# gfacciol/mgm

Hardware: AMD Instinct MI355X
Metric: disparity-volumes/sec (W*H*L cost volume -> 8-dir MGM -> WTA+vfit) (higher is better)
Workload: dtype f32

## Files before the change

### mgm_amd/csrc/mgm_wta.hip

```cpp
#include <algorithm>
#include <cstdlib>

#include "mgm_device.h"
#include "mgm_planner.h"

namespace mgm {

__device__ __forceinline__ void vfit(float v0, float v1, float v2, float &v_min, float &x_min)
{
    if ((v1 > v0) && (v1 > v2)) {
        v_min = v1;
        x_min = 0.0f;
        return;
    }
    float slope = v2 - v1;
    if ((v2 - v1) < (v0 - v1)) slope = v0 - v1;
    x_min = (v0 - v2) / (2.0f * slope);
    v_min = v2 + (x_min - 1.0f) * slope;
}

template <int LPL, int PPW, bool EXACT, int MAXD = kMaxDirs, int SUB = 1>
__global__ void __launch_bounds__(256) k_wta(const WtaParams P)
{
    static_assert(SUB == 1 || EXACT, "several pixels per slab only without padding lanes");
    constexpr int LP = LPL * 64;
    constexpr int LANES = 64 / SUB;
    __shared__ float sS[4][LP];
    const int wv = threadIdx.x >> 6, lane = threadIdx.x & 63;
    const int L = P.L;
    const int Lr_ = P.Lreal;
    constexpr bool exact = EXACT;
    const int Ls = SUB > 1 ? LP : L;
    const int m0 = lane * LPL;
    const int sub = lane / LANES;
    const int o0 = (lane % LANES) * LPL;
    const bool c8 = P.C8 && exact;
    const long long nslab = P.npix / SUB;
    for (long long g0 = ((long long)blockIdx.x * 4 + wv) * PPW; g0 < nslab; g0 += (long long)gridDim.x * 4 * PPW) {
        float c[PPW][LPL], l[MAXD][PPW][LPL];
#pragma unroll
        for (int u = 0; u < PPW; u++) {
            const long long g = g0 + u < nslab ? g0 + u : nslab - 1;
            if (c8 && P.cbytes == 2) {
                const unsigned short *q = reinterpret_cast<const unsigned short *>(P.C8) + g * Ls + m0;
#pragma unroll
                for (int k = 0; k < LPL; k++) c[u][k] = c16_decode(q[k]);
            } else if (c8) {
                const uint8_t *q = P.C8 + g * Ls + m0;
#pragma unroll
                for (int k = 0; k < LPL; k++) c[u][k] = c8_decode(q[k]);
            } else {
                const float *q = P.C + g * Ls + m0;
#pragma unroll
                for (int k = 0; k < LPL; k++) c[u][k] = (exact || m0 + k < L) ? q[k] : f_inf();
            }
        }
#pragma unroll
        for (int p = 0; p < MAXD; p++) {
            if (p < P.NDIR) {
#pragma unroll
                for (int u = 0; u < PPW; u++) {
                    const long long g = g0 + u < nslab ? g0 + u : nslab - 1;
                    const float *q = P.Lr + (long long)p * P.nvol + g * Ls + m0;
#pragma unroll
                    for (int k = 0; k < LPL; k++) l[p][u][k] = (exact || m0 + k < L) ? q[k] : f_inf();
                }
            }
        }
#pragma unroll
        for (int u = 0; u < PPW; u++) {
            if (g0 + u >= nslab) break;
            const long long pix = (g0 + u) * SUB + sub;
            float S[LPL];
#pragma unroll
            for (int k = 0; k < LPL; k++) S[k] = 0.0f;
#pragma unroll
            for (int p = 0; p < MAXD; p++) {
                if (p < P.NDIR) {
#pragma unroll
                    for (int k = 0; k < LPL; k++) S[k] = S[k] + l[p][u][k];
                }
            }
            if (P.FIX == 1) {
                const float f = (float)(P.NDIR - 1);
#pragma unroll
                for (int k = 0; k < LPL; k++) S[k] = S[k] - f * c[u][k];
            }
            float vout = 0.0f;
            if (P.FIX == 1) vout = vout - (float)(P.NDIR - 1) * f_inf();
            if (P.clo) {
                const int cl = (int)P.clo[pix] - P.dmin, ch = (int)P.chi[pix] - P.dmin;
#pragma unroll
                for (int k = 0; k < LPL; k++)
                    if (o0 + k < cl || o0 + k > ch) S[k] = vout;
            }
            if (P.S) {
                float *q = P.S + pix * Lr_ + o0;
#pragma unroll
                for (int k = 0; k < LPL; k++)
                    if (o0 + k < Lr_) q[k] = S[k];
            }
            float best = f_inf();
            int bi = 0x7fffffff;
            const bool windowed = P.wlo != nullptr;
            int wl = 0, wh = 0;
            if (windowed) {
                wl = (int)P.wlo[pix] - P.dmin;
                wh = (int)P.whi[pix] - P.dmin;
            }
#pragma unroll
            for (int k = 0; k < LPL; k++) {
                const float v = S[k];
                if (o0 + k < Lr_ && (!windowed || (o0 + k >= wl && o0 + k <= wh)) && finite_bits(v) && best > v) {
                    best = v;
                    bi = o0 + k;
                }
            }
#pragma unroll
            for (int d = LANES / 2; d >= 1; d >>= 1) {
                const float ov = __shfl_xor(best, d);
                const int oi = __shfl_xor(bi, d);
                if (ov < best || (ov == best && oi < bi)) {
                    best = ov;
                    bi = oi;
                }
            }
            if (windowed) {
                if (finite_bits(vout)) {
                    if (wl < 0 && wl <= wh && !(best < vout)) {
                        best = vout;
                        bi = wl;
                    }
                    const int hi0 = wl > Lr_ ? wl : Lr_;
                    if (wh >= Lr_ && hi0 <= wh && vout < best) {
                        best = vout;
                        bi = hi0;
                    }
                }
            }
            float outv, outc = best;
            if (bi == 0x7fffffff) outv = __builtin_nanf("");
            else outv = (float)(bi + P.dmin);
            if (P.refine == 1 && !windowed) {
#pragma unroll
                for (int k = 0; k < LPL; k++) sS[wv][m0 + k] = S[k];
                asm volatile("s_waitcnt lgkmcnt(0)" ::: "memory");
                if (bi != 0x7fffffff && bi - 1 >= 0 && bi + 2 <= Lr_ - 1) {
                    const float *sp = sS[wv] + sub * L;
                    const float v0 = sp[bi - 1], v1 = sp[bi], v2 = sp[bi + 1];
                    float vmin, dx;
                    vfit(v0, v1, v2, vmin, dx);
                    outv = (float)(bi + P.dmin) + dx;
                    outc = vmin;
                }
                asm volatile("s_waitcnt lgkmcnt(0)" ::: "memory");
            }
            if (lane % LANES == 0) {
                P.out[pix] = outv;
                P.outcost[pix] = outc;
            }
        }
    }
}

template <int L, int MAXD>
__global__ void __launch_bounds__(256) k_wta_q(const WtaParams P)
{
    static_assert(L == 192 || L == 384, "groups of 768 floats");
    constexpr int NPX = 768 / L;
    constexpr int CPP = L / 4;
    __shared__ float sS[4][768];
    const int wv = threadIdx.x >> 6, lane = threadIdx.x & 63;
    const bool c8 = P.C8 != nullptr;
    const long long ngroup = P.npix / NPX;
    int cpix[3], clab[3];
#pragma unroll
    for (int j = 0; j < 3; j++) {
        const int t = 64 * j + lane;
        cpix[j] = t / CPP;
        clab[j] = (t % CPP) * 4;
    }
    for (long long g = (long long)blockIdx.x * 4 + wv; g < ngroup; g += (long long)gridDim.x * 4) {
        float c[3][4], l[MAXD][3][4];
#pragma unroll
        for (int j = 0; j < 3; j++) {
            if (c8 && P.cbytes == 2) {
                const uint2 w = *reinterpret_cast<const uint2 *>(P.C8 + (g * 768 + 256 * j + 4 * lane) * 2);
                c[j][0] = c16_decode(w.x & 65535u); c[j][1] = c16_decode(w.x >> 16);
                c[j][2] = c16_decode(w.y & 65535u); c[j][3] = c16_decode(w.y >> 16);
            } else if (c8) {
                const unsigned w = *reinterpret_cast<const unsigned *>(P.C8 + g * 768 + 256 * j + 4 * lane);
#pragma unroll
                for (int k = 0; k < 4; k++) c[j][k] = c8_decode((w >> (8 * k)) & 255u);
            } else {
                const float4 q = *reinterpret_cast<const float4 *>(P.C + g * 768 + 256 * j + 4 * lane);
                c[j][0] = q.x; c[j][1] = q.y; c[j][2] = q.z; c[j][3] = q.w;
            }
        }
#pragma unroll
        for (int p = 0; p < MAXD; p++)
            if (p < P.NDIR) {
#pragma unroll
                for (int j = 0; j < 3; j++) {
                    const float4 q = *reinterpret_cast<const float4 *>(P.Lr + (long long)p * P.nvol + g * 768 + 256 * j + 4 * lane);
                    l[p][j][0] = q.x; l[p][j][1] = q.y; l[p][j][2] = q.z; l[p][j][3] = q.w;
                }
            }
        float S[3][4];
        const float f = (float)(P.NDIR - 1);
#pragma unroll
        for (int j = 0; j < 3; j++)
#pragma unroll
            for (int k = 0; k < 4; k++) {
                float a = 0.0f;
#pragma unroll
                for (int p = 0; p < MAXD; p++)
                    if (p < P.NDIR) a = a + l[p][j][k];
                if (P.FIX == 1) a = a - f * c[j][k];
                S[j][k] = a;
            }
        if (P.S) {
#pragma unroll
            for (int j = 0; j < 3; j++) *reinterpret_cast<float4 *>(P.S + g * 768 + 256 * j + 4 * lane) = make_float4(S[j][0], S[j][1], S[j][2], S[j][3]);
        }
        float cb[3];
        int ci[3];
#pragma unroll
        for (int j = 0; j < 3; j++) {
            cb[j] = f_inf();
            ci[j] = 0x7fffffff;
#pragma unroll
            for (int k = 0; k < 4; k++)
                if (finite_bits(S[j][k]) && cb[j] > S[j][k]) {
                    cb[j] = S[j][k];
                    ci[j] = clab[j] + k;
                }
        }
        if (P.refine == 1) {
#pragma unroll
            for (int j = 0; j < 3; j++) *reinterpret_cast<float4 *>(&sS[wv][256 * j + 4 * lane]) = make_float4(S[j][0], S[j][1], S[j][2], S[j][3]);
        }
#pragma unroll
        for (int q = 0; q < NPX; q++) {
            float best = f_inf();
            int bi = 0x7fffffff;
#pragma unroll
            for (int j = 0; j < 3; j++)
                if (cpix[j] == q && (cb[j] < best)) {
                    best = cb[j];
                    bi = ci[j];
                }
#pragma unroll
            for (int d = 32; d >= 1; d >>= 1) {
                const float ov = __shfl_xor(best, d);
                const int oi = __shfl_xor(bi, d);
                if (ov < best || (ov == best && oi < bi)) {
                    best = ov;
                    bi = oi;
                }
            }
            float outv, outc = best;
            if (bi == 0x7fffffff) outv = __builtin_nanf("");
            else outv = (float)(bi + P.dmin);
            if (P.refine == 1) {
                asm volatile("s_waitcnt lgkmcnt(0)" ::: "memory");
                if (bi != 0x7fffffff && bi - 1 >= 0 && bi + 2 <= L - 1) {
                    const float *sp = sS[wv] + q * L;
                    float vmin, dx;
                    vfit(sp[bi - 1], sp[bi], sp[bi + 1], vmin, dx);
                    outv = (float)(bi + P.dmin) + dx;
                    outc = vmin;
                }
            }
            if (lane == 0) {
                P.out[g * NPX + q] = outv;
                P.outcost[g * NPX + q] = outc;
            }
        }
        if (P.refine == 1) asm volatile("s_waitcnt lgkmcnt(0)" ::: "memory");
    }
}

__global__ void __launch_bounds__(256) k_wta_any(const WtaParams P)
{
    const int wv = threadIdx.x >> 6, lane = threadIdx.x & 63;
    const int L = P.L, Lr_ = P.Lreal;
    const float f = (float)(P.NDIR - 1);
    float vout = 0.0f;
    if (P.FIX == 1) vout = vout - f * f_inf();
    for (long long pix = (long long)blockIdx.x * 4 + wv; pix < P.npix; pix += (long long)gridDim.x * 4) {
        int cl = 0, ch = Lr_ - 1;
        if (P.clo) {
            cl = (int)P.clo[pix] - P.dmin;
            ch = (int)P.chi[pix] - P.dmin;
        }
        const bool windowed = P.wlo != nullptr;
        int wl = 0, wh = 0;
        if (windowed) {
            wl = (int)P.wlo[pix] - P.dmin;
            wh = (int)P.whi[pix] - P.dmin;
        }
        auto S_at = [&](int o) {
            float a = 0.0f;
            for (int p = 0; p < P.NDIR; p++) a = a + P.Lr[(long long)p * P.nvol + pix * L + o];
            if (P.FIX == 1)
                a = a - f * (!P.C8 ? P.C[pix * L + o]
                                   : (P.cbytes == 2 ? c16_decode(reinterpret_cast<const unsigned short *>(P.C8)[pix * L + o]) : c8_decode(P.C8[pix * L + o])));
            if (o < cl || o > ch) a = vout;
            return a;
        };
        float best = f_inf();
        int bi = 0x7fffffff;
        for (int o = lane; o < Lr_; o += 64) {
            const float v = S_at(o);
            if (P.S) P.S[pix * Lr_ + o] = v;
            if ((!windowed || (o >= wl && o <= wh)) && finite_bits(v) && best > v) {
                best = v;
                bi = o;
            }
        }
#pragma unroll
        for (int d = 32; d >= 1; d >>= 1) {
            const float ov = __shfl_xor(best, d);
            const int oi = __shfl_xor(bi, d);
            if (ov < best || (ov == best && oi < bi)) {
                best = ov;
                bi = oi;
            }
        }
        if (windowed && finite_bits(vout)) {
            if (wl < 0 && wl <= wh && !(best < vout)) {
                best = vout;
                bi = wl;
            }
            const int hi0 = wl > Lr_ ? wl : Lr_;
            if (wh >= Lr_ && hi0 <= wh && vout < best) {
                best = vout;
                bi = hi0;
            }
        }
        float outv, outc = best;
        if (bi == 0x7fffffff) outv = __builtin_nanf("");
        else outv = (float)(bi + P.dmin);
        if (P.refine == 1 && !windowed && bi != 0x7fffffff && bi - 1 >= 0 && bi + 2 <= Lr_ - 1) {
            float vmin, dx;
            vfit(S_at(bi - 1), S_at(bi), S_at(bi + 1), vmin, dx);
            outv = (float)(bi + P.dmin) + dx;
            outc = vmin;
        }
        if (lane == 0) {
            P.out[pix] = outv;
            P.outcost[pix] = outc;
        }
    }
}

template <int MAXD>
__device__ __forceinline__ void sum_fix(const float (&l)[MAXD][4], const float (&c)[4], int ndir, int fix, float (&S)[4])
{
#pragma unroll
    for (int k = 0; k < 4; k++) S[k] = 0.0f;
#pragma unroll
    for (int p = 0; p < MAXD; p++)
        if (p < ndir) {
#pragma unroll
            for (int k = 0; k < 4; k++) S[k] = S[k] + l[p][k];
        }
    if (fix == 1) {
        const float f = (float)(ndir - 1);
#pragma unroll
        for (int k = 0; k < 4; k++) S[k] = S[k] - f * c[k];
    }
}
template <int CTRL>
__device__ __forceinline__ float dpp_fmin(float v)
{
    return __builtin_fminf(v, __builtin_bit_cast(float, __builtin_amdgcn_update_dpp(0, __builtin_bit_cast(int, v), CTRL, 0xf, 0xf, false)));
}
template <int PPW, int MAXD, bool ALLD>
__global__ void __launch_bounds__(256) k_wta_pruned(const WtaParams P)
{
    constexpr int L = 256;
    __shared__ float sS[4][PPW][L];
    const int wv = threadIdx.x >> 6, lane = threadIdx.x & 63;
    const int ch = lane >> 3;
    const int o0 = lane * 4;
    const int ndir = ALLD ? MAXD : P.NDIR, fix = P.FIX;
    const long long mstride = P.nvol / 32;
    unsigned nloaded = 0, npx = 0;
    for (long long g0 = ((long long)blockIdx.x * 4 + wv) * PPW; g0 < P.npix; g0 += (long long)gridDim.x * 4 * PPW) {
        unsigned cw[PPW];
        float mn[PPW][MAXD];
#pragma unroll
        for (int u = 0; u < PPW; u++) {
            const long long pix = g0 + u < P.npix ? g0 + u : P.npix - 1;
            cw[u] = *reinterpret_cast<const unsigned *>(P.C8 + pix * L + o0);
#pragma unroll
            for (int p = 0; p < MAXD; p++)
                if (p < ndir) mn[u][p] = P.Lmin[(long long)p * mstride + pix * (L / 32) + ch];
        }
        float c[PPW][4], clb[PPW];
        int seed[PPW];
#pragma unroll
        for (int u = 0; u < PPW; u++) {
            float lm[MAXD][4], LB[4];
#pragma unroll
            for (int k = 0; k < 4; k++) c[u][k] = c8_decode((cw[u] >> (8 * k)) & 255u);
#pragma unroll
            for (int p = 0; p < MAXD; p++)
#pragma unroll
                for (int k = 0; k < 4; k++) lm[p][k] = p < ndir ? mn[u][p] : 0.0f;
            sum_fix<MAXD>(lm, c[u], ndir, fix, LB);
            float lb = f_inf();
#pragma unroll
            for (int k = 0; k < 4; k++) lb = c[u][k] < f_inf() ? __builtin_fminf(lb, LB[k]) : lb;
            lb = lb == lb ? lb : -f_inf();
            lb = dpp_fmin<0xB1>(lb);
            lb = dpp_fmin<0x4E>(lb);
            lb = dpp_fmin<0x141>(lb);
            clb[u] = lb;
            const float gmin = wave_min(lb);
            const unsigned long long at = __builtin_amdgcn_ballot_w64(lb == gmin);
            seed[u] = gmin < f_inf() ? (int)(__builtin_ctzll(at) >> 3) : -1;
        }
        float S[PPW][4];
        bool act[PPW];
        float best0[PPW];
        {
            float l[PPW][MAXD][4];
#pragma unroll
            for (int u = 0; u < PPW; u++) {
                const long long pix = g0 + u < P.npix ? g0 + u : P.npix - 1;
                act[u] = ch == seed[u];
                const float *q0 = P.Lr + pix * L + (seed[u] > 0 ? seed[u] : 0) * 32 + (lane & 7) * 4;
#pragma unroll
                for (int p = 0; p < MAXD; p++)
                    if (p < ndir) {
                        const float4 q = *reinterpret_cast<const float4 *>(q0 + (long long)p * P.nvol);
                        l[u][p][0] = q.x, l[u][p][1] = q.y, l[u][p][2] = q.z, l[u][p][3] = q.w;
                    }
            }
#pragma unroll
            for (int u = 0; u < PPW; u++) {
                sum_fix<MAXD>(l[u], c[u], ndir, fix, S[u]);
                float b = f_inf();
#pragma unroll
                for (int k = 0; k < 4; k++) b = (act[u] && finite_bits(S[u][k]) && S[u][k] < b) ? S[u][k] : b;
                best0[u] = wave_min(b);
            }
        }
        bool act2[PPW];
        {
            float l[PPW][MAXD][4];
#pragma unroll
            for (int u = 0; u < PPW; u++) {
                const long long pix = g0 + u < P.npix ? g0 + u : P.npix - 1;
                act2[u] = !act[u] && seed[u] >= 0 && clb[u] <= best0[u];
                const float *q0 = P.Lr + pix * L + (act2[u] ? ch : (seed[u] > 0 ? seed[u] : 0)) * 32 + (lane & 7) * 4;
#pragma unroll
                for (int p = 0; p < MAXD; p++)
                    if (p < ndir) {
                        const float4 q = *reinterpret_cast<const float4 *>(q0 + (long long)p * P.nvol);
                        l[u][p][0] = q.x, l[u][p][1] = q.y, l[u][p][2] = q.z, l[u][p][3] = q.w;
                    }
            }
#pragma unroll
            for (int u = 0; u < PPW; u++) {
                float S2[4];
                sum_fix<MAXD>(l[u], c[u], ndir, fix, S2);
#pragma unroll
                for (int k = 0; k < 4; k++) S[u][k] = act[u] ? S[u][k] : S2[k];
            }
        }
#pragma unroll
        for (int u = 0; u < PPW; u++) {
            if (g0 + u >= P.npix) break;
            const long long pix = g0 + u;
            const bool have = act[u] || act2[u];
            const unsigned long long lmask = __builtin_amdgcn_ballot_w64(have);
            nloaded += (unsigned)__builtin_popcountll(lmask & 0x0101010101010101ull);
            npx++;
            float best = f_inf();
            int bi = 0x7fffffff;
            if (have) {
#pragma unroll
                for (int k = 0; k < 4; k++)
                    if (finite_bits(S[u][k]) && best > S[u][k]) {
                        best = S[u][k];
                        bi = o0 + k;
                    }
            }
            const float gbest = wave_min(best);
            const unsigned long long who = __builtin_amdgcn_ballot_w64(bi != 0x7fffffff && best == gbest);
            best = gbest;
            bi = who ? __builtin_amdgcn_readlane(bi, (int)__builtin_ctzll(who)) : 0x7fffffff;
            float outv, outc = best;
            if (bi == 0x7fffffff) outv = __builtin_nanf("");
            else outv = (float)(bi + P.dmin);
            if (P.refine == 1) {
                if (have) {
#pragma unroll
                    for (int k = 0; k < 4; k++) sS[wv][u][o0 + k] = S[u][k];
                }
                if (bi != 0x7fffffff && bi - 1 >= 0 && bi + 2 <= L - 1) {
                    auto S_at = [&](int o) -> float {
                        if ((lmask >> ((o >> 5) * 8)) & 1ull) return sS[wv][u][o];
                        float a = 0.0f;
                        for (int p = 0; p < ndir; p++) a = a + P.Lr[(long long)p * P.nvol + pix * L + o];
                        if (fix == 1) a = a - (float)(ndir - 1) * c8_decode(P.C8[pix * L + o]);
                        return a;
                    };
                    const float v0 = S_at(bi - 1), v1 = S_at(bi), v2 = S_at(bi + 1);
                    float vmin, dx;
                    vfit(v0, v1, v2, vmin, dx);
                    outv = (float)(bi + P.dmin) + dx;
                    outc = vmin;
                }
            }
            if (lane == 0) {
                P.out[pix] = outv;
                P.outcost[pix] = outc;
            }
        }
    }
    if (P.stats && lane == 0) atomicAdd(P.stats + (blockIdx.x & 63) * 16, ((unsigned long long)npx << 32) | nloaded);
}

static_assert(kWtaWidestLabels == kMaxLPL * 64, "plan_wta sends wider volumes to k_wta_any");
hipError_t launch_wta(const WtaParams &p, const WtaChoice &c, hipStream_t s)
{
    const dim3 grid((unsigned)c.grid), block(256);
#define WTA(LPL_, PPW_, EXACT_, MAXD_, SUB_)                                                                     \
    if (c.LPL == LPL_ && c.PPW == PPW_ && c.EXACT == EXACT_ && c.MAXD == MAXD_ && c.SUB == SUB_) {               \
        hipLaunchKernelGGL((k_wta<LPL_, PPW_, EXACT_ != 0, MAXD_, SUB_>), grid, block, 0, s, p);                 \
        return hipGetLastError();                                                                                \
    }
#define WTA_Q(LPL_, MAXD_)                                                                                       \
    if (c.LPL == LPL_ && c.MAXD == MAXD_) {                                                                      \
        hipLaunchKernelGGL((k_wta_q<64 * LPL_, MAXD_>), grid, block, 0, s, p);                                   \
        return hipGetLastError();                                                                                \
    }
#define WTA_PRUNED(PPW_, MAXD_, ALLD_)                                                                           \
    if (c.PPW == PPW_ && c.MAXD == MAXD_ && c.ALLD == ALLD_) {                                                   \
        hipLaunchKernelGGL((k_wta_pruned<PPW_, MAXD_, ALLD_ != 0>), grid, block, 0, s, p);                       \
        return hipGetLastError();                                                                                \
    }
    switch (c.family) {
        case kWtaPruned:
            if (!p.Lmin) break;
            WTA_PRUNED(2, 8, 1) WTA_PRUNED(1, 8, 1) WTA_PRUNED(2, 4, 1) WTA_PRUNED(1, 4, 1) WTA_PRUNED(1, 4, 0) WTA_PRUNED(1, 8, 0)
            break;
        case kWtaAny:
            hipLaunchKernelGGL(k_wta_any, grid, block, 0, s, p);
            return hipGetLastError();
        case kWtaQuad:
            WTA_Q(3, 4) WTA_Q(3, 8) WTA_Q(6, 4) WTA_Q(6, 8)
            break;
        case kWtaPacked:
            WTA(4, 4, 1, 4, 2) WTA(4, 2, 1, 8, 2) WTA(4, 4, 1, 4, 4) WTA(4, 2, 1, 8, 4)
            break;
        case kWtaPlain:
            WTA(1, 8, 1, 4, 1) WTA(1, 4, 1, 8, 1) WTA(1, 1, 0, 8, 1)
            WTA(2, 8, 1, 4, 1) WTA(2, 4, 1, 8, 1) WTA(2, 1, 0, 8, 1)
            WTA(3, 4, 1, 4, 1) WTA(3, 2, 1, 8, 1) WTA(3, 1, 0, 8, 1)
            WTA(4, 6, 1, 4, 1) WTA(4, 3, 1, 8, 1) WTA(4, 1, 0, 8, 1)
            WTA(6, 2, 1, 4, 1) WTA(6, 1, 1, 8, 1) WTA(6, 1, 0, 8, 1)
            WTA(8, 2, 1, 4, 1) WTA(8, 1, 1, 8, 1) WTA(8, 1, 0, 8, 1)
            WTA(12, 1, 1, 8, 1) WTA(12, 1, 0, 8, 1)
            WTA(16, 1, 1, 8, 1) WTA(16, 1, 0, 8, 1)
            WTA(24, 1, 0, 8, 1)
            WTA(32, 1, 0, 8, 1)
            break;
        default: break;
    }
#undef WTA
#undef WTA_Q
#undef WTA_PRUNED
    return hipErrorInvalidValue;
}

__device__ __forceinline__ void parabolafit(const float (&v)[4], float &v_min, float &x_min)
{
    if (v[1] > v[0] && v[1] > v[2]) {
        x_min = 0;
        v_min = v[1];
        return;
    }
    const float c = v[1];
    const float b = (v[2] - v[0]) / 2;
    const float a = (v[2] - 2 * v[1] + v[0]) / 2;
    float x = -b / (2 * a);
    if (x > 1) x = 1;
    if (x < -1) x = -1;
    v_min = (a * x + b) * x + c;
    x_min = x;
}

__device__ __forceinline__ void parabolafit_ocv(const float (&v)[4], float &v_min, float &x_min)
{
    if (v[1] > v[0] && v[1] > v[2]) {
        x_min = 0;
        v_min = v[1];
        return;
    }
    const float c = v[1];
    float b = (v[2] - v[0]) / 2;
    float a = (v[2] - 2 * v[1] + v[0]) / 2;
    a *= 2;
    b *= 2;
    a = a > 1.0 ? a : 1.0;
    float x = (-b + a) / (2 * a);
    if (x > 1) x = 1;
    if (x < -1) x = -1;
    v_min = (a * x + b) * x + c;
    x_min = x;
}

__device__ __forceinline__ float cubic_interp(const float (&p)[4], const float x)
{
    return p[1] + 0.5 * x *
                      (p[2] - p[0] + x * (2.0 * p[0] - 5.0 * p[1] + 4.0 * p[2] - p[3] + x * (3.0 * (p[1] - p[2]) + p[3] - p[0])));
}

__device__ __forceinline__ void cubicfit(const float (&p)[4], float &out_pmin, float &out_xmin)
{
    float pmin, xmin;
    if (p[1] < p[2]) {
        pmin = p[1];
        xmin = 0.0;
    } else {
        pmin = p[2];
        xmin = 1.0;
    }
    const double a = 0.5 * 3.0 * (3.0 * (p[1] - p[2]) + p[3] - p[0]);
    const double b = 2.0 * p[0] - 5.0 * p[1] + 4.0 * p[2] - p[3];
    const double c = 0.5 * (p[2] - p[0]);
    const double discr = b * b - 4.0 * a * c;
    if (discr >= 0) {
        const double z1 = (-b + __builtin_sqrt(discr)) / (2.0 * a);
        const double z2 = (-b - __builtin_sqrt(discr)) / (2.0 * a);
        if (z1 > 0.0 && z1 < 1.0) {
            const float tmp = cubic_interp(p, z1);
            if (tmp < pmin) {
                pmin = tmp;
                xmin = z1;
            }
        }
        if (z2 > 0.0 && z2 < 1.0) {
            const float tmp = cubic_interp(p, z2);
            if (tmp < pmin) {
                pmin = tmp;
                xmin = z2;
            }
        }
    }
    out_pmin = pmin;
    out_xmin = xmin;
}

template <int SPL, int CB>
__global__ void __launch_bounds__(256) k_wta_rel(const WtaRelParams P)
{
    constexpr int SLOTS = 16 * SPL;
    const int wv = threadIdx.x >> 6, lane = threadIdx.x & 63, li = lane & 15, grp = lane >> 4;
    const float f = (float)(P.NDIR - 1);
    float vout = 0.0f;
    if (P.FIX == 1) vout = vout - f * f_inf();
    const bool vfin = finite_bits(vout);
    const long long nquads = (P.npix + 3) / 4;
    for (long long q4 = (long long)blockIdx.x * 4 + wv; q4 < nquads; q4 += (long long)gridDim.x * 4) {
        const long long pix0 = q4 * 4 + grp;
        const bool live = pix0 < P.npix;
        const long long pix = live ? pix0 : P.npix - 1;
        const int4 rec = reinterpret_cast<const int4 *>(P.base)[pix];
        const int b = rec.x, lo = rec.y, hi = rec.z;
        const bool windowed = P.wlo != nullptr;
        const int wl = windowed ? (int)P.wlo[pix] : lo, wh = windowed ? (int)P.whi[pix] : hi;
        typedef float f4 __attribute__((ext_vector_type(4)));
        float a[SPL];
#pragma unroll
        for (int q = 0; q < SPL; q++) a[q] = 0.0f;
        for (int p = 0; p < P.NDIR; p++) {
#pragma unroll
            for (int h = 0; h < SPL / 4; h++) {
                const f4 t = reinterpret_cast<const f4 *>(P.Lr + (long long)p * P.nvol + pix * SLOTS + SPL * li)[h];
#pragma unroll
                for (int q = 0; q < 4; q++) a[4 * h + q] = a[4 * h + q] + t[q];
            }
        }
        if (P.FIX == 1) {
            constexpr int NWORD = SPL * CB / 4;
            unsigned cw[NWORD];
#pragma unroll
            for (int w = 0; w < NWORD; w++) cw[w] = reinterpret_cast<const unsigned *>(P.c8 + (pix * SLOTS + SPL * li) * CB)[w];
#pragma unroll
            for (int q = 0; q < SPL; q++)
                a[q] = a[q] - f * (CB == 1 ? c8_decode((cw[q / 4] >> (8 * (q % 4))) & 255u)
                                           : (CB == 2 ? c16_decode((cw[q / 2] >> (16 * (q % 2))) & 65535u) : __builtin_bit_cast(float, cw[q * CB / 4])));
        }
        float val[SPL];
        float cb = f_inf();
        int ci = 0x7fffffff;
#pragma unroll
        for (int q = 0; q < SPL; q++) {
            const int d = b + SPL * li + q;
            const bool own = d >= lo && d <= hi;
            val[q] = own ? a[q] : vout;
            if (own && d >= wl && d <= wh && finite_bits(val[q]) && val[q] < cb) {
                cb = val[q];
                ci = d;
            }
        }
        auto take = [&](float ov, int oi) {
            if (ov < cb || (ov == cb && oi < ci)) {
                cb = ov;
                ci = oi;
            }
        };
        take(__builtin_bit_cast(float, __builtin_amdgcn_update_dpp(0, __builtin_bit_cast(int, cb), 0xB1, 0xf, 0xf, false)), __builtin_amdgcn_update_dpp(0, ci, 0xB1, 0xf, 0xf, false));
        take(__builtin_bit_cast(float, __builtin_amdgcn_update_dpp(0, __builtin_bit_cast(int, cb), 0x4E, 0xf, 0xf, false)), __builtin_amdgcn_update_dpp(0, ci, 0x4E, 0xf, 0xf, false));
        take(__builtin_bit_cast(float, __builtin_amdgcn_update_dpp(0, __builtin_bit_cast(int, cb), 0x141, 0xf, 0xf, false)), __builtin_amdgcn_update_dpp(0, ci, 0x141, 0xf, 0xf, false));
        take(__builtin_bit_cast(float, __builtin_amdgcn_update_dpp(0, __builtin_bit_cast(int, cb), 0x140, 0xf, 0xf, false)), __builtin_amdgcn_update_dpp(0, ci, 0x140, 0xf, 0xf, false));
        float best = f_inf();
        int bi = 0x7fffffff;
        if (wl < lo && wl <= wh && vfin) {
            best = vout;
            bi = wl;
        }
        if (ci != 0x7fffffff && best > cb) {
            best = cb;
            bi = ci;
        }
        const int hi0 = wl > hi + 1 ? wl : hi + 1;
        if (wh > hi && hi0 <= wh && vfin && vout < best) {
            best = vout;
            bi = hi0;
        }
        float outv, outc = best;
        if (bi == 0x7fffffff) outv = __builtin_nanf("");
        else outv = (float)bi;
        float v[4];
#pragma unroll
        for (int k = 0; k < 4; k++) {
            const int sl = (bi == 0x7fffffff ? b : bi) - 1 + k - b;
            const int e = sl & (SPL - 1);
            float mine = val[0];
#pragma unroll
            for (int q = 1; q < SPL; q++) mine = e == q ? val[q] : mine;
            const float x = __shfl(mine, (lane & 48) | ((sl / SPL) & 15));
            v[k] = (sl >= 0 && sl < SLOTS) ? x : vout;
        }
        if (P.refine >= 1 && bi != 0x7fffffff && bi - 1 >= wl && bi + 2 <= wh) {
            float vmin = outc, dx = 0;
            if (P.refine == 1) vfit(v[0], v[1], v[2], vmin, dx);
            else if (P.refine == 2) parabolafit(v, vmin, dx);
            else if (P.refine == 3) cubicfit(v, vmin, dx);
            else parabolafit_ocv(v, vmin, dx);
            outv = (float)bi + dx;
            outc = vmin;
        }
        if (li == 0 && live) {
            P.out[pix] = outv;
            P.outcost[pix] = outc;
        }
    }
}
__global__ void __launch_bounds__(256) k_rel_S(const WtaRelParams P, long long n, int L, int dmin, float *__restrict__ S)
{
    const long long t = (long long)blockIdx.x * blockDim.x + threadIdx.x;
    if (t >= n) return;
    const long long pix = t / L;
    const int d = dmin + (int)(t - pix * L);
    const int4 rec = reinterpret_cast<const int4 *>(P.base)[pix];
    const float f = (float)(P.NDIR - 1);
    float s = f_inf();
    if (d >= rec.y && d <= rec.z) {
        const long long k = pix * P.slots + (d - rec.x);
        s = 0.0f;
        for (int p = 0; p < P.NDIR; p++) s = s + P.Lr[(long long)p * P.nvol + k];
        if (P.FIX == 1)
            s = s - f * (P.cb == 1 ? c8_decode((unsigned)P.c8[k])
                                   : (P.cb == 2 ? c16_decode((unsigned)reinterpret_cast<const uint16_t *>(P.c8)[k]) : reinterpret_cast<const float *>(P.c8)[k]));
    } else if (P.FIX == 1)
        s = s - f * f_inf();
    S[t] = s;
}
hipError_t launch_rel_S(const WtaRelParams &p, int L, int dmin, float *S, hipStream_t s)
{
    const long long n = p.npix * L;
    hipLaunchKernelGGL(k_rel_S, dim3((unsigned)((n + 255) / 256)), dim3(256), 0, s, p, n, L, dmin, S);
    return hipGetLastError();
}
hipError_t launch_wta_rel(const WtaRelParams &p, hipStream_t s)
{
    const WtaRelChoice c = plan_wta_rel(WtaRelRequest{p.npix, p.num_cu, p.slots, p.cb});
    const dim3 grid((unsigned)c.grid);
#define WTA_REL(SPL_, CB_)                                                                \
    if (c.SPL == SPL_ && c.CB == CB_) {                                                   \
        hipLaunchKernelGGL((k_wta_rel<SPL_, CB_>), grid, dim3(256), 0, s, p);             \
        return hipGetLastError();                                                         \
    }
    WTA_REL(8, 4) WTA_REL(8, 2) WTA_REL(8, 1) WTA_REL(4, 4) WTA_REL(4, 2) WTA_REL(4, 1)
#undef WTA_REL
    return hipErrorInvalidValue;
}

__global__ void __launch_bounds__(256) k_refine(const float *__restrict__ S, long long npix, int L, int dmin, int method,
                                                const float *__restrict__ wlo, const float *__restrict__ whi, float vout,
                                                float *__restrict__ out, float *__restrict__ outcost)
{
    const long long i = (long long)blockIdx.x * blockDim.x + threadIdx.x;
    if (i >= npix) return;
    const float minP = out[i];
    if (!(minP == minP)) return;
    const int o = (int)minP;
    const int lo = wlo ? (int)wlo[i] : dmin, hi = whi ? (int)whi[i] : dmin + L - 1;
    if (o - 1 >= lo && o + 2 <= hi) {
        const float *Si = S + i * L;
        float v[4];
#pragma unroll
        for (int k = 0; k < 4; k++) {
            const int d = o - 1 + k - dmin;
            v[k] = (d >= 0 && d < L) ? Si[d] : vout;
        }
        float vmin = outcost[i], dx = 0;
        if (method == 1) vfit(v[0], v[1], v[2], vmin, dx);
        else if (method == 2) parabolafit(v, vmin, dx);
        else if (method == 3) cubicfit(v, vmin, dx);
        else parabolafit_ocv(v, vmin, dx);
        out[i] = (float)o + dx;
        outcost[i] = vmin;
    }
}

hipError_t launch_refine(const float *S, long long npix, int L, int dmin, int method, const float *wlo, const float *whi,
                         float vout, float *out, float *outcost, hipStream_t s)
{
    if (method < 1 || method > 4) return hipErrorInvalidValue;
    hipLaunchKernelGGL(k_refine, dim3((unsigned)((npix + 255) / 256)), dim3(256), 0, s, S, npix, L, dmin, method, wlo, whi, vout,
                       out, outcost);
    return hipGetLastError();
}

__device__ __forceinline__ float right_cost_at(const WtaRightParams &P, long long i)
{
    if (!P.C8) return P.C[i];
    return P.cbytes == 2 ? c16_decode(reinterpret_cast<const unsigned short *>(P.C8)[i]) : c8_decode(P.C8[i]);
}
__device__ __forceinline__ float right_S_at(const WtaRightParams &P, int y, int xr, int oR)
{
    const int x = xr + oR - P.dmax;
    if (x < 0 || x >= P.nx) return f_inf();
    const long long i = ((long long)y * P.nx + x) * P.Lk + (P.L - 1 - oR);
    float a = 0.0f;
    for (int p = 0; p < P.NDIR; p++) a = a + P.Lr[(long long)p * P.nvol + i];
    if (P.FIX == 1) a = a - (float)(P.NDIR - 1) * right_cost_at(P, i);
    return a;
}
__device__ __forceinline__ void right_emit(const WtaRightParams &P, int y, int xr, int oR, float v1)
{
    float outv = __builtin_nanf(""), outc = f_inf();
    if (oR >= 0) {
        outv = (float)(oR - P.dmax);
        outc = v1;
        if (P.refine == 1 && oR - 1 >= 0 && oR + 2 <= P.L - 1) {
            float vmin, dx;
            vfit(right_S_at(P, y, xr, oR - 1), v1, right_S_at(P, y, xr, oR + 1), vmin, dx);
            outv = (float)(oR - P.dmax) + dx;
            outc = vmin;
        }
    }
    const long long i = (long long)y * P.vnx + xr;
    P.out[i] = outv;
    P.outcost[i] = outc;
}

template <int LPL, int PPW>
__global__ void __launch_bounds__(256) k_wta_right(const WtaRightParams P)
{
    constexpr int CH = 4 * PPW;
    extern __shared__ unsigned long long ring[];
    const int tid = threadIdx.x, wv = tid >> 6, lane = tid & 63;
    const int nseg = (P.vnx + P.seg - 1) / P.seg;
    const int y = blockIdx.x / nseg;
    const int xr0 = (blockIdx.x % nseg) * P.seg, xr1 = min(xr0 + P.seg, P.vnx);
    const int xlo = max(0, xr0 - P.dmax), xhi = min(P.nx, xr1 - P.dmin);
    const unsigned mask = (unsigned)P.ring - 1u;
    const int o0 = lane * LPL;
    const bool c8 = P.C8 != nullptr;
    for (int i = tid; i < P.ring; i += 256) ring[i] = ~0ull;
    int fin = xr0;
    if (xlo < xhi) {
        const int first = max(xr0, xlo + P.dmin);
        for (int xr = xr0 + tid; xr < first; xr += 256) right_emit(P, y, xr, -1, 0.0f);
        fin = first;
        __syncthreads();
        for (int xa = xlo; xa < xhi; xa += CH) {
            const int xb = min(xa + CH, xhi);
            float c[PPW][LPL], l[kMaxDirs][PPW][LPL];
#pragma unroll
            for (int u = 0; u < PPW; u++) {
                const int x = min(xa + wv * PPW + u, xhi - 1);
                const long long g = ((long long)y * P.nx + x) * (64 * LPL) + o0;
                if (P.FIX != 1) {
#pragma unroll
                    for (int k = 0; k < LPL; k++) c[u][k] = 0.0f;
                } else if (c8 && P.cbytes == 2) {
                    const unsigned short *q = reinterpret_cast<const unsigned short *>(P.C8) + g;
#pragma unroll
                    for (int k = 0; k < LPL; k++) c[u][k] = c16_decode(q[k]);
                } else if (c8) {
                    const uint8_t *q = P.C8 + g;
#pragma unroll
                    for (int k = 0; k < LPL; k++) c[u][k] = c8_decode(q[k]);
                } else {
                    const float *q = P.C + g;
#pragma unroll
                    for (int k = 0; k < LPL; k++) c[u][k] = q[k];
                }
            }
#pragma unroll
            for (int p = 0; p < kMaxDirs; p++) {
                if (p < P.NDIR) {
#pragma unroll
                    for (int u = 0; u < PPW; u++) {
                        const int x = min(xa + wv * PPW + u, xhi - 1);
                        const float *q = P.Lr + (long long)p * P.nvol + ((long long)y * P.nx + x) * (64 * LPL) + o0;
#pragma unroll
                        for (int k = 0; k < LPL; k++) l[p][u][k] = q[k];
                    }
                }
            }
#pragma unroll
            for (int u = 0; u < PPW; u++) {
                const int x = xa + wv * PPW + u;
                if (x >= xhi) break;
                float S[LPL];
#pragma unroll
                for (int k = 0; k < LPL; k++) S[k] = 0.0f;
#pragma unroll
                for (int p = 0; p < kMaxDirs; p++) {
                    if (p < P.NDIR) {
#pragma unroll
                        for (int k = 0; k < LPL; k++) S[k] = S[k] + l[p][u][k];
                    }
                }
                if (P.FIX == 1) {
                    const float f = (float)(P.NDIR - 1);
#pragma unroll
                    for (int k = 0; k < LPL; k++) S[k] = S[k] - f * c[u][k];
                }
#pragma unroll
                for (int k = 0; k < LPL; k++) {
                    const int o = o0 + k, xr = x + P.dmin + o;
                    if (o < P.L && xr >= xr0 && xr < xr1 && finite_bits(S[k])) {
                        const unsigned long long key = ((unsigned long long)f2ord(S[k]) << 32) | (unsigned)(P.L - 1 - o);
                        atomicMin(&ring[(unsigned)xr & mask], key);
                    }
                }
            }
            __syncthreads();
            const int fe = min(xr1, xb == xhi ? xhi + P.dmax : xb + P.dmin);
            for (int i = lane * 4 + wv; fin + i < fe; i += 256) {
                const int xr = fin + i;
                const unsigned long long key = ring[(unsigned)xr & mask];
                ring[(unsigned)xr & mask] = ~0ull;
                if (key == ~0ull) right_emit(P, y, xr, -1, 0.0f);
                else right_emit(P, y, xr, (int)(unsigned)key, ord2f((unsigned)(key >> 32)));
            }
            fin = max(fin, fe);
        }
    }
    for (int xr = fin + tid; xr < xr1; xr += 256) right_emit(P, y, xr, -1, 0.0f);
}

__global__ void __launch_bounds__(256) k_wta_right_any(const WtaRightParams P)
{
    const int wv = threadIdx.x >> 6, lane = threadIdx.x & 63;
    const long long npix = (long long)P.vnx * P.ny;
    for (long long pix = (long long)blockIdx.x * 4 + wv; pix < npix; pix += (long long)gridDim.x * 4) {
        const int y = (int)(pix / P.vnx), xr = (int)(pix % P.vnx);
        float best = f_inf();
        int bi = 0x7fffffff;
        for (int oR = lane; oR < P.L; oR += 64) {
            const float v = right_S_at(P, y, xr, oR);
            if (finite_bits(v) && best > v) {
                best = v;
                bi = oR;
            }
        }
#pragma unroll
        for (int d = 32; d >= 1; d >>= 1) {
            const float ov = __shfl_xor(best, d);
            const int oi = __shfl_xor(bi, d);
            if (ov < best || (ov == best && oi < bi)) {
                best = ov;
                bi = oi;
            }
        }
        if (lane == 0) right_emit(P, y, xr, bi == 0x7fffffff ? -1 : bi, best);
    }
}

hipError_t launch_wta_right(const WtaRightParams &p0, const WtaRightChoice &c, hipStream_t s)
{
    const dim3 grid((unsigned)c.grid), block(256);
    if (c.family == kRightDiagonal) {
        hipLaunchKernelGGL(k_wta_right_any, grid, block, 0, s, p0);
        return hipGetLastError();
    }
    if (c.family != kRightStream) return hipErrorInvalidValue;
    WtaRightParams p = p0;
    p.seg = c.seg;
    p.ring = c.ring;
    const size_t lds = sizeof(unsigned long long) * (size_t)c.ring;
#define WTA_RIGHT(LPL_, PPW_)                                                             \
    if (c.LPL == LPL_ && c.PPW == PPW_) {                                                 \
        hipLaunchKernelGGL((k_wta_right<LPL_, PPW_>), grid, block, lds, s, p);            \
        return hipGetLastError();                                                         \
    }
    WTA_RIGHT(1, 2) WTA_RIGHT(2, 2) WTA_RIGHT(3, 2) WTA_RIGHT(4, 2) WTA_RIGHT(6, 1) WTA_RIGHT(8, 1) WTA_RIGHT(12, 1) WTA_RIGHT(16, 1)
#undef WTA_RIGHT
    return hipErrorInvalidValue;
}

}
```

Measured before the change: 160.7.

## Remap pruned WTA to one pixel per 8-lane group with iterative candidate chunks

The pruned WTA kernel used to assign a whole 64-lane wave to each pixel. It now gives each 8-lane group its own pixel, so a wave covers 8 pixels per step. Lower bounds are computed per chunk from the max cost code, and the wave loops over candidate chunks until none remain, replacing the fixed two-pass load. Subpixel refinement reads the three neighbours directly and combines them with DPP instead of staging through shared memory, and NDIR becomes a compile-time template parameter. This aims to cut cross-lane reductions and wasted lanes per pixel, at the cost of possible divergence in the candidate loop and a looser lower bound.

```diff
diff --git a/mgm_amd/csrc/mgm_wta.hip b/mgm_amd/csrc/mgm_wta.hip
--- a/mgm_amd/csrc/mgm_wta.hip
+++ b/mgm_amd/csrc/mgm_wta.hip
@@ -355,175 +355,226 @@
     }
 }
 
-template <int MAXD>
-__device__ __forceinline__ void sum_fix(const float (&l)[MAXD][4], const float (&c)[4], int ndir, int fix, float (&S)[4])
-{
-#pragma unroll
-    for (int k = 0; k < 4; k++) S[k] = 0.0f;
+template <int MAXD, int K>
+__device__ __forceinline__ void sum_fix(const float (&l)[MAXD][K], const float (&c)[K], int ndir, int fix, float (&S)[K])
+{
+#pragma unroll
+    for (int k = 0; k < K; k++) S[k] = 0.0f;
 #pragma unroll
     for (int p = 0; p < MAXD; p++)
         if (p < ndir) {
 #pragma unroll
-            for (int k = 0; k < 4; k++) S[k] = S[k] + l[p][k];
+            for (int k = 0; k < K; k++) S[k] = S[k] + l[p][k];
         }
     if (fix == 1) {
         const float f = (float)(ndir - 1);
 #pragma unroll
-        for (int k = 0; k < 4; k++) S[k] = S[k] - f * c[k];
-    }
+        for (int k = 0; k < K; k++) S[k] = S[k] - f * c[k];
+    }
+}
+template <int CTRL>
+__device__ __forceinline__ float dpp_f(float v)
+{
+    return __builtin_bit_cast(float, __builtin_amdgcn_update_dpp(0, __builtin_bit_cast(int, v), CTRL, 0xf, 0xf, false));
 }
 template <int CTRL>
 __device__ __forceinline__ float dpp_fmin(float v)
 {
-    return __builtin_fminf(v, __builtin_bit_cast(float, __builtin_amdgcn_update_dpp(0, __builtin_bit_cast(int, v), CTRL, 0xf, 0xf, false)));
+    return __builtin_fminf(v, dpp_f<CTRL>(v));
+}
+__device__ __forceinline__ float group_fmin(float v)
+{
+    v = dpp_fmin<0xB1>(v);
+    v = dpp_fmin<0x4E>(v);
+    return dpp_fmin<0x141>(v);
+}
+template <int CTRL>
+__device__ __forceinline__ void dpp_take(float &best, int &bi)
+{
+    const float ov = dpp_f<CTRL>(best);
+    const int oi = __builtin_amdgcn_update_dpp(0, bi, CTRL, 0xf, 0xf, false);
+    if (ov < best || (ov == best && oi < bi)) {
+        best = ov;
+        bi = oi;
+    }
+}
+template <int PPW, int ND>
+__device__ __forceinline__ void wta_pruned(const WtaParams &P)
+{
+    constexpr int MAXD = ND;
+    constexpr int L = 256;
+    constexpr int NONE = 0x7fffffff;
+    const int wv = threadIdx.x >> 6, lane = threadIdx.x & 63;
+    const int j = lane & 7;
+    const int gsh = lane & ~7;
+    const int ndir = ND, fix = P.FIX;
+    const long long mstride = P.nvol / 32;
+    unsigned nloaded = 0, npx = 0;
+    for (long long g0 = ((long long)blockIdx.x * 4 + wv) * (8 * PPW); g0 < P.npix; g0 += (long long)gridDim.x * 4 * 8 * PPW) {
+        long long pix[PPW];
+        bool own[PPW];
+        uint4 cq[PPW][2];
+        float mn[PPW][MAXD];
+#pragma unroll
+        for (int u = 0; u < PPW; u++) {
+            const long long q = g0 + 8 * u + (lane >> 3);
+            own[u] = q < P.npix;
+            pix[u] = own[u] ? q : P.npix - 1;
+            const uint4 *cp = reinterpret_cast<const uint4 *>(P.C8 + pix[u] * L + j * 32);
+            cq[u][0] = cp[0], cq[u][1] = cp[1];
+#pragma unroll
+            for (int p = 0; p < MAXD; p++)
+                if (p < ndir) mn[u][p] = P.Lmin[(long long)p * mstride + pix[u] * (L / 32) + j];
+        }
+        float clb[PPW];
+        int seed[PPW];
+#pragma unroll
+        for (int u = 0; u < PPW; u++) {
+            const unsigned w[8] = {cq[u][0].x, cq[u][0].y, cq[u][0].z, cq[u][0].w, cq[u][1].x, cq[u][1].y, cq[u][1].z, cq[u][1].w};
+            unsigned m = 0;
+#pragma unroll
+            for (int i = 0; i < 8; i++)
+#pragma unroll
+                for (int k = 0; k < 4; k++) m = max(m, (((w[i] >> (8 * k)) & 255u) + 1u) & 255u);
+            float lm[MAXD][1], LB[1];
+            const float cm[1] = {(float)((int)m - 1)};
+#pragma unroll
+            for (int p = 0; p < MAXD; p++) lm[p][0] = p < ndir ? mn[u][p] : 0.0f;
+            sum_fix<MAXD>(lm, cm, ndir, fix, LB);
+            const float lb = (m != 0u && LB[0] == LB[0]) ? LB[0] : f_inf();
+            clb[u] = lb;
+            const float gmin = group_fmin(lb);
+            const unsigned at = (unsigned)(__builtin_amdgcn_ballot_w64(lb == gmin) >> gsh) & 255u;
+            seed[u] = gmin < f_inf() ? __builtin_ctz(at | 256u) : -1;
+        }
+        auto chunk_S = [&](const int (&ck)[PPW], float (&S)[PPW][4]) {
+            float l[PPW][MAXD][4];
+            unsigned cw[PPW];
+#pragma unroll
+            for (int u = 0; u < PPW; u++) {
+                const long long at = pix[u] * L + ck[u] * 32 + j * 4;
+                cw[u] = *reinterpret_cast<const unsigned *>(P.C8 + at);
+#pragma unroll
+                for (int p = 0; p < MAXD; p++)
+                    if (p < ndir) {
+                        const float4 q = *reinterpret_cast<const float4 *>(P.Lr + (long long)p * P.nvol + at);
+                        l[u][p][0] = q.x, l[u][p][1] = q.y, l[u][p][2] = q.z, l[u][p][3] = q.w;
+                    }
+            }
+#pragma unroll
+            for (int u = 0; u < PPW; u++) {
+                float c[4];
+#pragma unroll
+                for (int k = 0; k < 4; k++) c[k] = c8_decode((cw[u] >> (8 * k)) & 255u);
+                sum_fix<MAXD>(l[u], c, ndir, fix, S[u]);
+            }
+        };
+        float best[PPW];
+        int bi[PPW], sck[PPW];
+        unsigned cand[PPW];
+        {
+            float S[PPW][4];
+#pragma unroll
+            for (int u = 0; u < PPW; u++) sck[u] = seed[u] > 0 ? seed[u] : 0;
+            chunk_S(sck, S);
+#pragma unroll
+            for (int u = 0; u < PPW; u++) {
+                best[u] = f_inf();
+                bi[u] = NONE;
+                if (seed[u] >= 0) {
+#pragma unroll
+                    for (int k = 0; k < 4; k++)
+                        if (finite_bits(S[u][k]) && best[u] > S[u][k]) {
+                            best[u] = S[u][k];
+                            bi[u] = seed[u] * 32 + j * 4 + k;
+                        }
+                }
+                const float best0 = group_fmin(best[u]);
+                const bool cd = seed[u] >= 0 && j != seed[u] && clb[u] <= best0;
+                const unsigned long long cdm = __builtin_amdgcn_ballot_w64(cd);
+                cand[u] = (unsigned)(cdm >> gsh) & 255u;
+                const unsigned long long ownm = __builtin_amdgcn_ballot_w64(own[u]);
+                nloaded += (unsigned)__builtin_popcountll(cdm & ownm) + (unsigned)__builtin_popcountll(__builtin_amdgcn_ballot_w64(own[u] && j == seed[u]));
+                npx += (unsigned)__builtin_popcountll(ownm) >> 3;
+            }
+        }
+        for (;;) {
+            bool more = false;
+#pragma unroll
+            for (int u = 0; u < PPW; u++) more = more || cand[u] != 0u;
+            if (!__builtin_amdgcn_ballot_w64(more)) break;
+            if (more) {
+                int ck[PPW];
+                float S[PPW][4];
+#pragma unroll
+                for (int u = 0; u < PPW; u++) ck[u] = cand[u] != 0u ? __builtin_ctz(cand[u]) : sck[u];
+                chunk_S(ck, S);
+#pragma unroll
+                for (int u = 0; u < PPW; u++)
+                    if (cand[u] != 0u) {
+#pragma unroll
+                        for (int k = 0; k < 4; k++) {
+                            const int o = ck[u] * 32 + j * 4 + k;
+                            if (finite_bits(S[u][k]) && (S[u][k] < best[u] || (S[u][k] == best[u] && o < bi[u]))) {
+                                best[u] = S[u][k];
+                                bi[u] = o;
+                            }
+                        }
+                        cand[u] &= cand[u] - 1u;
+                    }
+            }
+        }
+#pragma unroll
+        for (int u = 0; u < PPW; u++) {
+            dpp_take<0xB1>(best[u], bi[u]);
+            dpp_take<0x4E>(best[u], bi[u]);
+            dpp_take<0x141>(best[u], bi[u]);
+            const int b = bi[u];
+            float outv, outc = best[u];
+            if (b == NONE) outv = __builtin_nanf("");
+            else outv = (float)(b + P.dmin);
+            if (P.refine == 1) {
+                const bool gate = b != NONE && b - 1 >= 0 && b + 2 <= L - 1;
+                float a = 0.0f;
+                if (gate && j < 3) {
+                    const long long at = pix[u] * L + (b - 1 + j);
+#pragma unroll
+                    for (int p = 0; p < MAXD; p++)
+                        if (p < ndir) a = a + P.Lr[(long long)p * P.nvol + at];
+                    if (fix == 1) a = a - (float)(ndir - 1) * c8_decode(P.C8[at]);
+                }
+                const float v1 = dpp_f<0xB1>(a), v2 = dpp_f<0x4E>(a);
+                if (gate) {
+                    float vmin, dx;
+                    vfit(a, v1, v2, vmin, dx);
+                    outv = (float)(b + P.dmin) + dx;
+                    outc = vmin;
+                }
+            }
+            if (j == 0 && own[u]) {
+                P.out[pix[u]] = outv;
+                P.outcost[pix[u]] = outc;
+            }
+        }
+    }
+    if (P.stats && lane == 0) atomicAdd(P.stats + (blockIdx.x & 63) * 16, ((unsigned long long)npx << 32) | nloaded);
 }
 template <int PPW, int MAXD, bool ALLD>
 __global__ void __launch_bounds__(256) k_wta_pruned(const WtaParams P)
 {
-    constexpr int L = 256;
-    __shared__ float sS[4][PPW][L];
-    const int wv = threadIdx.x >> 6, lane = threadIdx.x & 63;
-    const int ch = lane >> 3;
-    const int o0 = lane * 4;
-    const int ndir = ALLD ? MAXD : P.NDIR, fix = P.FIX;
-    const long long mstride = P.nvol / 32;
-    unsigned nloaded = 0, npx = 0;
-    for (long long g0 = ((long long)blockIdx.x * 4 + wv) * PPW; g0 < P.npix; g0 += (long long)gridDim.x * 4 * PPW) {
-        unsigned cw[PPW];
-        float mn[PPW][MAXD];
-#pragma unroll
-        for (int u = 0; u < PPW; u++) {
-            const long long pix = g0 + u < P.npix ? g0 + u : P.npix - 1;
-            cw[u] = *reinterpret_cast<const unsigned *>(P.C8 + pix * L + o0);
-#pragma unroll
-            for (int p = 0; p < MAXD; p++)
-                if (p < ndir) mn[u][p] = P.Lmin[(long long)p * mstride + pix * (L / 32) + ch];
-        }
-        float c[PPW][4], clb[PPW];
-        int seed[PPW];
-#pragma unroll
-        for (int u = 0; u < PPW; u++) {
-            float lm[MAXD][4], LB[4];
-#pragma unroll
-            for (int k = 0; k < 4; k++) c[u][k] = c8_decode((cw[u] >> (8 * k)) & 255u);
-#pragma unroll
-            for (int p = 0; p < MAXD; p++)
-#pragma unroll
-                for (int k = 0; k < 4; k++) lm[p][k] = p < ndir ? mn[u][p] : 0.0f;
-            sum_fix<MAXD>(lm, c[u], ndir, fix, LB);
-            float lb = f_inf();
-#pragma unroll
-            for (int k = 0; k < 4; k++) lb = c[u][k] < f_inf() ? __builtin_fminf(lb, LB[k]) : lb;
-            lb = lb == lb ? lb : -f_inf();
-            lb = dpp_fmin<0xB1>(lb);
-            lb = dpp_fmin<0x4E>(lb);
-            lb = dpp_fmin<0x141>(lb);
-            clb[u] = lb;
-            const float gmin = wave_min(lb);
-            const unsigned long long at = __builtin_amdgcn_ballot_w64(lb == gmin);
-            seed[u] = gmin < f_inf() ? (int)(__builtin_ctzll(at) >> 3) : -1;
-        }
-        float S[PPW][4];
-        bool act[PPW];
-        float best0[PPW];
-        {
-            float l[PPW][MAXD][4];
-#pragma unroll
-            for (int u = 0; u < PPW; u++) {
-                const long long pix = g0 + u < P.npix ? g0 + u : P.npix - 1;
-                act[u] = ch == seed[u];
-                const float *q0 = P.Lr + pix * L + (seed[u] > 0 ? seed[u] : 0) * 32 + (lane & 7) * 4;
-#pragma unroll
-                for (int p = 0; p < MAXD; p++)
-                    if (p < ndir) {
-                        const float4 q = *reinterpret_cast<const float4 *>(q0 + (long long)p * P.nvol);
-                        l[u][p][0] = q.x, l[u][p][1] = q.y, l[u][p][2] = q.z, l[u][p][3] = q.w;
-                    }
-            }
-#pragma unroll
-            for (int u = 0; u < PPW; u++) {
-                sum_fix<MAXD>(l[u], c[u], ndir, fix, S[u]);
-                float b = f_inf();
-#pragma unroll
-                for (int k = 0; k < 4; k++) b = (act[u] && finite_bits(S[u][k]) && S[u][k] < b) ? S[u][k] : b;
-                best0[u] = wave_min(b);
-            }
-        }
-        bool act2[PPW];
-        {
-            float l[PPW][MAXD][4];
-#pragma unroll
-            for (int u = 0; u < PPW; u++) {
-                const long long pix = g0 + u < P.npix ? g0 + u : P.npix - 1;
-                act2[u] = !act[u] && seed[u] >= 0 && clb[u] <= best0[u];
-                const float *q0 = P.Lr + pix * L + (act2[u] ? ch : (seed[u] > 0 ? seed[u] : 0)) * 32 + (lane & 7) * 4;
-#pragma unroll
-                for (int p = 0; p < MAXD; p++)
-                    if (p < ndir) {
-                        const float4 q = *reinterpret_cast<const float4 *>(q0 + (long long)p * P.nvol);
-                        l[u][p][0] = q.x, l[u][p][1] = q.y, l[u][p][2] = q.z, l[u][p][3] = q.w;
-                    }
-            }
-#pragma unroll
-            for (int u = 0; u < PPW; u++) {
-                float S2[4];
-                sum_fix<MAXD>(l[u], c[u], ndir, fix, S2);
-#pragma unroll
-                for (int k = 0; k < 4; k++) S[u][k] = act[u] ? S[u][k] : S2[k];
-            }
-        }
-#pragma unroll
-        for (int u = 0; u < PPW; u++) {
-            if (g0 + u >= P.npix) break;
-            const long long pix = g0 + u;
-            const bool have = act[u] || act2[u];
-            const unsigned long long lmask = __builtin_amdgcn_ballot_w64(have);
-            nloaded += (unsigned)__builtin_popcountll(lmask & 0x0101010101010101ull);
-            npx++;
-            float best = f_inf();
-            int bi = 0x7fffffff;
-            if (have) {
-#pragma unroll
-                for (int k = 0; k < 4; k++)
-                    if (finite_bits(S[u][k]) && best > S[u][k]) {
-                        best = S[u][k];
-                        bi = o0 + k;
-                    }
-            }
-            const float gbest = wave_min(best);
-            const unsigned long long who = __builtin_amdgcn_ballot_w64(bi != 0x7fffffff && best == gbest);
-            best = gbest;
-            bi = who ? __builtin_amdgcn_readlane(bi, (int)__builtin_ctzll(who)) : 0x7fffffff;
-            float outv, outc = best;
-            if (bi == 0x7fffffff) outv = __builtin_nanf("");
-            else outv = (float)(bi + P.dmin);
-            if (P.refine == 1) {
-                if (have) {
-#pragma unroll
-                    for (int k = 0; k < 4; k++) sS[wv][u][o0 + k] = S[u][k];
-                }
-                if (bi != 0x7fffffff && bi - 1 >= 0 && bi + 2 <= L - 1) {
-                    auto S_at = [&](int o) -> float {
-                        if ((lmask >> ((o >> 5) * 8)) & 1ull) return sS[wv][u][o];
-                        float a = 0.0f;
-                        for (int p = 0; p < ndir; p++) a = a + P.Lr[(long long)p * P.nvol + pix * L + o];
-                        if (fix == 1) a = a - (float)(ndir - 1) * c8_decode(P.C8[pix * L + o]);
-                        return a;
-                    };
-                    const float v0 = S_at(bi - 1), v1 = S_at(bi), v2 = S_at(bi + 1);
-                    float vmin, dx;
-                    vfit(v0, v1, v2, vmin, dx);
-                    outv = (float)(bi + P.dmin) + dx;
-                    outc = vmin;
-                }
-            }
-            if (lane == 0) {
-                P.out[pix] = outv;
-                P.outcost[pix] = outc;
-            }
-        }
-    }
-    if (P.stats && lane == 0) atomicAdd(P.stats + (blockIdx.x & 63) * 16, ((unsigned long long)npx << 32) | nloaded);
+    if constexpr (ALLD) {
+        wta_pruned<PPW, MAXD>(P);
+    } else {
+#define ND_CASE(N_)                                         \
+    case N_:                                                \
+        if constexpr (N_ < MAXD) wta_pruned<PPW, N_>(P);    \
+        break;
+        switch (P.NDIR) {
+            ND_CASE(1) ND_CASE(2) ND_CASE(3) ND_CASE(4) ND_CASE(5) ND_CASE(6) ND_CASE(7)
+            default: break;
+        }
+#undef ND_CASE
+    }
 }
 
 static_assert(kWtaWidestLabels == kMaxLPL * 64, "plan_wta sends wider volumes to k_wta_any");
@@ -541,7 +592,7 @@
         return hipGetLastError();                                                                                \
     }
 #define WTA_PRUNED(PPW_, MAXD_, ALLD_)                                                                           \
-    if (c.PPW == PPW_ && c.MAXD == MAXD_ && c.ALLD == ALLD_) {                                                   \
+    if (c.PPW == PPW_ && c.MAXD == MAXD_ && c.ALLD == ALLD_ && p.NDIR >= 1 && (ALLD_ ? p.NDIR == MAXD_ : p.NDIR < MAXD_)) { \
         hipLaunchKernelGGL((k_wta_pruned<PPW_, MAXD_, ALLD_ != 0>), grid, block, 0, s, p);                       \
         return hipGetLastError();                                                                                \
     }
```

After: 177.1 (median of 6 runs). +10.2%, better.
